# MP-Gadget/MP-Gadget

Hardware: AMD Instinct MI355X
Metric: particle-updates/sec (gravity force step: PM + tree build + short-range walk) (higher is better)
Workload: dtype f64

## Files before the change

include/mpgadget_hip.h:

```cpp
#ifndef MPGADGET_HIP_H
#define MPGADGET_HIP_H

#include <stddef.h>
#include <stdint.h>

#ifdef __cplusplus
extern "C" {
#endif

typedef struct mpg_engine mpg_engine;

int mpg_engine_create(mpg_engine **out, int device);
void mpg_engine_destroy(mpg_engine *eng);
const char *mpg_last_error(void);
const char *mpg_version(void);
const char *mpg_build_stamp(void);
int mpg_engine_set_stream(mpg_engine *eng, void *hip_stream);
void *mpg_engine_get_stream(mpg_engine *eng);
int mpg_engine_synchronize(mpg_engine *eng);

typedef struct mpg_gravshort_tree_params {
    double ErrTolForceAcc;
    double BHOpeningAngle;
    double MaxBHOpeningAngle;
// ... 295 lines not shown
int mpg_domain_local_refine(const uint64_t *keys, const int64_t *costs, int64_t nsample, mpg_topnode *tree, int *size, int MaxTopNodes, int *failed);
int mpg_domain_toptree_truncate(mpg_topnode *tree, int *size, int64_t countlimit, int64_t costlimit);
int mpg_domain_toptree_merge(mpg_topnode *A, int *sizeA, const mpg_topnode *B, int sizeB, int MaxTopNodes, int *failed);
int mpg_domain_global_refine(mpg_topnode *tree, int *size, int MaxTopNodes, int64_t countlimit, int64_t costlimit, int *failed);
int mpg_domain_create_topleaves(mpg_topnode *tree, int size, int *leaf_topnode, int *nleaves);
int mpg_domain_assign_topleaves_balanced(mpg_topnode *tree, int size, int *leaf_topnode, int nleaves, const int64_t *cost, int NTask,
                                         int NsegmentPerTask, int *leaf_task, int *StartLeaf, int *EndLeaf);
int mpg_dev_domain_topleaves(mpg_engine *eng, int64_t n, const double *d_pos, const unsigned char *d_garbage, double BoxSize,
                             const mpg_topnode *tree, int size, int nleaves, const int *leaf_task, int NTask, int32_t *d_topleaf,
                             int32_t *d_task, int64_t *leaf_counts, int64_t *task_counts);

int mpg_dev_peano_keys(mpg_engine *eng, int64_t n, const double *d_pos, double BoxSize, uint64_t *d_keys);
int mpg_dev_order_by_type_and_key(mpg_engine *eng, int64_t n, const unsigned char *d_type, const unsigned char *d_flags,
                                  const uint64_t *d_keys, int *d_perm, int64_t *n_live);

typedef struct mpg_fof_params {
    int FOFPrimaryLinkTypes;
    int FOFSecondaryLinkTypes;
    double FOFHaloComovingLinkingLength;
    int FOFHaloMinLength;
} mpg_fof_params;
typedef struct mpg_fof_groups {
    uint64_t *MinID;
    int *Length, *GrNr, *LenType;
    double *Mass, *MassType;
    double *CM, *Vel, *Jmom;
    double *Imom;
    float *FirstPos;
} mpg_fof_groups;
int mpg_dev_fof_fof(mpg_engine *eng, const mpg_fof_params *par, const uint64_t *d_id, const double *d_vel, const double *d_hsml,
                    const unsigned char *d_flags, int64_t *d_grnr, int64_t *ngroups);
int mpg_dev_fof_groups(mpg_engine *eng, const mpg_fof_groups *out);

typedef struct mpg_bigblock_info {
    char dtype[8];
    int nmemb;
    int nfile;
    int64_t size;
} mpg_bigblock_info;
int mpg_bigfile_block_info(const char *file, const char *block, mpg_bigblock_info *info);
int mpg_bigfile_read_block(const char *file, const char *block, int64_t start, int64_t count, const char *want_dtype, void *out);
int mpg_bigfile_write_block(const char *file, const char *block, const char *dtype, int nmemb, int nfile, int64_t size, const char *src_dtype,
                            const void *data);
int mpg_bigfile_get_attr(const char *file, const char *block, const char *name, const char *want_dtype, void *out, int nmemb);
int mpg_bigfile_set_attr(const char *file, const char *block, const char *name, const char *dtype, const void *data, int nmemb);

int mpg_gravpm_measure_power(mpg_engine *eng, int on);
int mpg_dev_gravpm_powerspectrum_raw(mpg_engine *eng, double *d_acc, int64_t *d_modes);
int mpg_powerspectrum_sum(int nbins, const double *acc, const int64_t *modes, double BoxSize_in_MPC, double *kk, double *Power,
                          int64_t *Nmodes, int *nonzero);
int mpg_gravpm_get_powerspectrum(mpg_engine *eng, double BoxSize_in_MPC, double *kk, double *Power, int64_t *Nmodes, int *nonzero);
int mpg_powerspectrum_save(const char *OutputDir, const char *filename, double Time, double D1, int nonzero, const double *kk,
                           const double *Power, const int64_t *Nmodes);

int mpg_dev_pm_slab_init(mpg_engine *eng, int rank, int world, int64_t *cplx_per_peer, int64_t *plane_doubles);

int mpg_dev_tree_top_partial(mpg_engine *eng, int La, int64_t n_own, double *d_out);
int mpg_dev_tree_top_set(mpg_engine *eng, int La, const double *d_sums);
int mpg_dev_pm_slab_forward_a(mpg_engine *eng, double *sendA);
int mpg_dev_pm_slab_forward_b(mpg_engine *eng, double *recvA, double *sendB);
int mpg_dev_pm_slab_inverse_c(mpg_engine *eng, const double *recvB, double *ghost_send);
int mpg_dev_pm_slab_readout(mpg_engine *eng, const double *ghost_recv, const int *d_targets, int64_t ntargets, double *d_gravpm,
                            double *d_potential);

typedef struct mpg_comm {
    void *ctx;
    int ThisTask, NTask;
    int device_buffers;
    int (*allreduce)(void *ctx, void *buf, int64_t count, int dtype, int op, int on_device);
    int (*alltoall_i64)(void *ctx, const int64_t *send, int64_t *recv);
    int (*alltoallv)(void *ctx, const void *send, const int64_t *sendbytes, const int64_t *sdispls, void *recv, const int64_t *recvbytes,
                     const int64_t *rdispls, int on_device);
    int (*bind_stream)(void *ctx, void *hip_stream);
} mpg_comm;

#define MPG_RCCL_ID_BYTES 128
typedef struct mpg_rccl mpg_rccl;
int mpg_rccl_available(void);
int mpg_rccl_get_unique_id(void *id128);
int mpg_rccl_create(mpg_rccl **out, int ThisTask, int NTask, const void *id128, int device);
int mpg_rccl_comm(mpg_rccl *r, mpg_comm *out);
int mpg_rccl_selftest(mpg_rccl *r, int64_t bytes_per_peer);
int mpg_rccl_stats(mpg_rccl *r, int64_t *calls3, int64_t *bytes_sent, int *version);
int mpg_rccl_comm_info(mpg_rccl *r, int *nranks, int *rank, int *device);
const char *mpg_rccl_last_error(mpg_rccl *r);
void mpg_rccl_destroy(mpg_rccl *r);

typedef struct mpg_dist mpg_dist;
int mpg_dist_create(mpg_dist **out, mpg_engine *eng, const mpg_comm *comm);
void mpg_dist_destroy(mpg_dist *d);
int mpg_dist_domain_decompose(mpg_dist *d, int64_t n, const double *d_pos, const unsigned char *d_garbage, double BoxSize,
                              int DomainOverDecompositionFactor, int DomainUseGlobalSorting, const float *d_cost, int *NTopNodes,
                              int *NTopLeaves);
int mpg_dist_domain_get(mpg_dist *d, mpg_topnode *TopNodes, int *leaf_task, int *StartLeaf, int *EndLeaf, int64_t *TopLeafCount);
int mpg_dist_domain_exchange(mpg_dist *d, int64_t n, int ncols, const void *const *d_cols, const int *col_bytes, int64_t *n_new,
                             void **d_new_cols);
int mpg_dist_use_decomposition(mpg_dist *d, double BoxSize, double margin, int La);
int mpg_dist_domain_maintain(mpg_dist *d, int64_t n, const double *d_pos, const unsigned char *d_garbage, double BoxSize, int64_t *n_leaving);
int mpg_dist_set_domain(mpg_dist *d, double BoxSize, const mpg_topnode *TopNodes, int NTopNodes, const int *leaf_task, int NTopLeaves,
                        double margin, int La);
int mpg_dist_gravity_step(mpg_dist *d, int64_t n_own, const double *d_pos, const float *d_mass, const double *d_oldacc,
                          const double *d_prev_accel, double *d_accel, double *d_gravpm, double *d_potential, double rho0);
int mpg_dist_dev_gravpm_force(mpg_dist *d, int64_t n_own, const double *d_pos, const float *d_mass, double *d_gravpm, double *d_potential);
int mpg_dist_dev_set_garbage(mpg_dist *d, int64_t n_own, const unsigned char *d_garbage);
int mpg_dist_dev_force_tree_build(mpg_dist *d, int64_t n_own, const double *d_pos, const float *d_mass);
int mpg_dist_dev_grav_short_tree(mpg_dist *d, const double *d_oldacc, const double *d_prev_accel, const double *d_gravpm, double *d_accel,
// ... 47 lines not shown
```

mp-gadget_amd/build.py:

```python
import hashlib
import os
import subprocess
import sys
from concurrent.futures import ThreadPoolExecutor

HERE = os.path.dirname(os.path.abspath(__file__))
CSRC = os.path.join(HERE, "csrc")
OBJ = os.path.join(CSRC, "_obj")
LIB = os.path.join(HERE, "libmpgadget_hip.so")
SOURCES = ["tree_build.hip", "grav_walk.hip", "grav_walk_coop.hip", "grav_walk_split.hip", "grav_pair_walk.hip", "pm.hip", "sph.hip", "timestep.hip", "peano.hip", "domain.hip", "fof.hip", "snapshot_io.hip", "engine.hip", "dist.hip", "rccl_comm.hip"]
HIPCC = os.environ.get("HIPCC", "/opt/rocm/bin/hipcc")
FLAGS = ["--offload-arch=gfx950", "-O3", "-std=c++17", "-fPIC", "-Wall", "-Wno-unused-function", "-Wno-unused-result"]
_EXTRA = os.environ.get("MPG_EXTRA_FLAGS", "")
_EXTRA_FILE, _EXTRA = (_EXTRA.split(":", 1) if ".hip:" in _EXTRA else ("", _EXTRA))


def _headers():
    hs = sorted(os.path.join(CSRC, f) for f in os.listdir(CSRC) if f.endswith(".h"))
    hs.append(os.path.join(HERE, "..", "include", "mpgadget_hip.h"))
    return hs


def _sha(paths, extra=""):
    h = hashlib.sha256(extra.encode())
    for p in paths:
        h.update(os.path.basename(p).encode())
        with open(p, "rb") as f:
            h.update(f.read())
    return h.hexdigest()


def source_stamp():
    return _sha([os.path.join(CSRC, s) for s in SOURCES] + _headers(), " ".join(FLAGS) + os.environ.get("MPG_EXTRA_FLAGS", ""))[:32]


def _read(path):
    try:
        with open(path) as f:
            return f.read().strip()
    except OSError:
        return ""


def build(force=False, verbose=False):
    os.makedirs(OBJ, exist_ok=True)
    headers = _headers()

    def compile_one(src):
        s = os.path.join(CSRC, src)
        o = os.path.join(OBJ, src.replace(".hip", ".o"))
        flags = FLAGS + (_EXTRA.split() if _EXTRA_FILE in ("", src) else [])
        want = _sha([s] + headers, " ".join(flags))
        if force or not os.path.exists(o) or _read(o + ".hash") != want:
            cmd = [HIPCC] + flags + ["-c", s, "-o", o]
            if verbose:
                print(" ".join(cmd))
            subprocess.check_call(cmd)
            with open(o + ".hash", "w") as f:
                f.write(want)
            return o, True
        return o, False

    with ThreadPoolExecutor(max_workers=4) as ex:
# ... 22 lines not shown
```

mp-gadget_amd/csrc/engine.hip:

```cpp
#include "engine_internal.h"
#include <atomic>
#include <chrono>
#include <cstdio>

static thread_local std::string g_err;
std::string &mpg_err_slot() { return g_err; }

extern "C" {

const char *mpg_last_error(void) { return g_err.c_str(); }
const char *mpg_version(void) { return "mpgadget_hip 0.1 (gfx950; TreePM gravity: PM + tree + short-range walk)"; }

int mpg_engine_create(mpg_engine **out, int device)
{
    API_BEGIN
    MPG_CHECK(out != nullptr, "mpg_engine_create: null output pointer");
    int ndev = 0;
    hipError_t e = hipGetDeviceCount(&ndev);
    if(e != hipSuccess || ndev <= 0)
        fail(__FILE__, __LINE__, "mpg_engine_create: no HIP device available (this engine has no CPU path)");
    MPG_CHECK(device >= 0 && device < ndev, "mpg_engine_create: bad device index");
    MPG_HIP(hipSetDevice(device));
    mpg_engine *eng = new mpg_engine();
    eng->device = device;
// ... 191 lines not shown
    API_BEGIN
    MPG_CHECK(eng, "null engine");
    MPG_CHECK(n >= 0 && (n == 0 || (d_pos && d_mass)), "mpg_dev_bind_particles: null particle arrays");
    MPG_CHECK(BoxSize > 0, "mpg_dev_bind_particles: BoxSize must be positive");
    eng->host_join();
    eng->n = n;
    eng->d_pos = d_pos;
    eng->d_mass = d_mass;
    eng->d_type = d_type;
    eng->box = BoxSize;
    eng->pm_queued = false;
    API_END
}

int mpg_dev_gravpm_force(mpg_engine *eng, double *d_gravpm, double *d_potential)
{
    API_BEGIN
    MPG_CHECK(eng && d_gravpm, "null argument");
    MPG_HIP(hipSetDevice(eng->device));
    MPG_CHECK(eng->pm.nmesh > 0, "gravpm_force called before gravpm_init_periodic");
    MPG_CHECK(eng->pm.box == eng->box, "gravpm_force: BoxSize of the mesh differs from the bound particles");
    static const bool no_overlap = getenv("MPG_NO_TREE_OVERLAP") != nullptr;
    if(!no_overlap && !eng->timer.enabled) {
        if(!eng->aux_stream) {
            MPG_HIP(hipStreamCreateWithFlags(&eng->aux_stream, hipStreamNonBlocking));
            MPG_HIP(hipEventCreateWithFlags(&eng->ev_inputs, hipEventDisableTiming));
            MPG_HIP(hipEventCreateWithFlags(&eng->ev_tree_done, hipEventDisableTiming));
            MPG_HIP(hipEventCreateWithFlags(&eng->ev_pad_done, hipEventDisableTiming));
        }
        MPG_HIP(hipEventRecord(eng->ev_inputs, eng->stream));
        eng->pm_queued = true;
    }
    eng->pm.force(eng->n, eng->d_pos, eng->d_mass, nullptr, d_gravpm, d_potential, eng->stream, &eng->timer);
    API_END
}

int mpg_dev_tree_top_partial(mpg_engine *eng, int La, int64_t n_own, double *d_out)
{
    API_BEGIN
    MPG_CHECK(eng && d_out, "null argument");
    MPG_CHECK(eng->tree_allocated, "no tree");
    MPG_HIP(hipSetDevice(eng->device));
    eng->tree.top_partial(La, n_own, d_out, eng->stream);
    API_END
}

int mpg_dev_tree_top_set(mpg_engine *eng, int La, const double *d_sums)
{
    API_BEGIN
    MPG_CHECK(eng && d_sums, "null argument");
    MPG_CHECK(eng->tree_allocated, "no tree");
    MPG_HIP(hipSetDevice(eng->device));
    eng->tree.top_set(La, d_sums, eng->stream);
    API_END
}

int mpg_dev_pm_slab_init(mpg_engine *eng, int rank, int world, int64_t *cplx_per_peer, int64_t *plane_doubles)
{
    API_BEGIN
    MPG_CHECK(eng, "null engine");
    MPG_HIP(hipSetDevice(eng->device));
    eng->pm.slab_init(rank, world);
    if(cplx_per_peer)
        *cplx_per_peer = (int64_t)eng->pm.slab_cplx_per_peer();
    if(plane_doubles)
        *plane_doubles = (int64_t)eng->pm.nmesh * eng->pm.nmesh;
    API_END
}

int mpg_dev_pm_slab_forward_a(mpg_engine *eng, double *sendA)
{
    API_BEGIN
    MPG_CHECK(eng && sendA, "null argument");
    MPG_HIP(hipSetDevice(eng->device));
    MPG_CHECK(eng->pm.box == eng->box, "gravpm_force: BoxSize of the mesh differs from the bound particles");
    eng->pm.slab_forward_a(eng->n, eng->d_pos, eng->d_mass, sendA, eng->stream);
    API_END
}

int mpg_dev_pm_slab_forward_b(mpg_engine *eng, double *recvA, double *sendB)
{
    API_BEGIN
    MPG_CHECK(eng && recvA && sendB, "null argument");
    MPG_HIP(hipSetDevice(eng->device));
    eng->pm.slab_forward_b(recvA, sendB, eng->stream);
    API_END
}

int mpg_dev_pm_slab_inverse_c(mpg_engine *eng, const double *recvB, double *ghost_send)
{
    API_BEGIN
    MPG_CHECK(eng && recvB && ghost_send, "null argument");
    MPG_HIP(hipSetDevice(eng->device));
    eng->pm.slab_inverse_c(recvB, ghost_send, eng->stream);
    API_END
}

int mpg_dev_pm_slab_readout(mpg_engine *eng, const double *ghost_recv, const int *d_targets, int64_t ntargets, double *d_gravpm,
                            double *d_potential)
{
    API_BEGIN
    MPG_CHECK(eng && ghost_recv && d_gravpm && (d_targets || ntargets == 0), "null argument");
    MPG_HIP(hipSetDevice(eng->device));
    eng->pm.slab_readout(ghost_recv, d_targets, ntargets, eng->d_pos, d_gravpm, d_potential, eng->stream);
    API_END
}
// ... 2769 lines not shown
```

mp-gadget_amd/csrc/pm.h:

```cpp
#pragma once
#include "mpg_common.h"
#include "tree_build.h"
#include <rocfft/rocfft.h>
#include <vector>

namespace mpg {

struct FftPlan {
    rocfft_plan plan = nullptr;
    rocfft_execution_info info = nullptr;
    DevBuf<char> work;
    void create(rocfft_result_placement placement, rocfft_transform_type type, int dims, const size_t *lengths, size_t batch,
                const size_t *in_strides = nullptr, size_t in_dist = 0, const size_t *out_strides = nullptr, size_t out_dist = 0);
    void exec(void *in, void *out, hipStream_t st);
    void destroy();
    bool ready() const { return plan != nullptr; }
};

struct PMesh {
    double box = 0, Asmth = 0, G = 0, cellsize = 0;
    int nmesh = 0;
    bool have_plans = false;
    bool kspace_force = false;
    FftPlan plan_r2c, plan_c2r;
    DevBuf<double> real;
    DevBuf<double> rho_k;
    DevBuf<double> work_k;
    DevBuf<double> grad_z;
    DevBuf<double> invsinc2, difffac;
    struct DepositState {
        int mode = 0, since_tune = 0;
    } dep_single, dep_slab;
    void deposit(int64_t n, const double *d_pos, const float *d_mass, const uint8_t *d_active, double *mesh, int x0, int P, DepositState &ds,
                 hipStream_t st, EventTimer *tm);
    DevBuf<unsigned long long> dep_keys_a, dep_keys_b;
    DevBuf<int> dep_idx_a, dep_idx_b;
    DevBuf<char> dep_tmp;
    bool measure_power = true, ps_valid = false;
    DevBuf<double> ps_acc;
    DevBuf<unsigned long long> ps_modes;
    void ps_zero(hipStream_t st);
    size_t ps_lds_bytes() const { return (size_t)nmesh * 3 * sizeof(double); }

    void init(double BoxSize, double Asmth, int Nmesh, double G, hipStream_t st);
    void ensure_single();
    void destroy();
    void force(int64_t n, const double *d_pos, const float *d_mass, const uint8_t *d_active, double *d_gravpm, double *d_potential,
               hipStream_t st, EventTimer *tm);
    ~PMesh() { destroy(); }

    struct Slab {
        int rank = 0, world = 1, P = 0, Py = 0;
        bool ready = false;
        FftPlan p2d_r2c, p2d_c2r, p1d_fwd, p1d_inv, p1d_fwd_t, p1d_inv_t;
        bool strided = false;
        DevBuf<double> phi;
        DevBuf<double> force;
        DevBuf<double> C;
        DevBuf<double> rho_k;
        DevBuf<double> work;
    } slab;
    DevBuf<unsigned> slab_err;
    size_t slab_cplx_per_peer() const { return (size_t)slab.P * slab.Py * (nmesh / 2 + 1); }
    void slab_init(int rank, int world);
    void slab_destroy();
    void slab_forward_a(int64_t n, const double *d_pos, const float *d_mass, double *sendA, hipStream_t st);
    void slab_forward_b(double *recvA, double *sendB, hipStream_t st);
    void slab_inverse_c(const double *recvB, double *ghost_send, hipStream_t st);
    void slab_readout_rows(const double *ghost_recv, int64_t nrows, const double *d_pos, double *d_gravpm, double *d_potential, hipStream_t st);
    void slab_readout(const double *ghost_recv, const int *targets, int64_t nt, const double *d_pos, double *d_gravpm, double *d_potential,
                      hipStream_t st);
};

}
```

mp-gadget_amd/csrc/pm.hip:

```cpp
#include "pm.h"
#include <cmath>
#include <cstdlib>
#include <cstring>
#include <rocprim/rocprim.hpp>

namespace mpg {

#define MPG_FFT(expr)                                                                                          \
    do {                                                                                                       \
        rocfft_status _r = (expr);                                                                             \
        if(_r != rocfft_status_success)                                                                        \
            ::mpg::fail(__FILE__, __LINE__, std::string("rocFFT error ") + std::to_string((int)_r) + " in " #expr); \
    } while(0)

__device__ __forceinline__ int wrap(int i, int n)
{
    i = (i >= n) ? i - n : i;
    i = (i < 0) ? i + n : i;
    return i;
}

__global__ void __launch_bounds__(256) k_cic_deposit(int64_t n, const double *__restrict__ pos, const float *__restrict__ mass,
                                                     const uint8_t *__restrict__ active, double cellsize, int nmesh,
                                                     double *__restrict__ mesh)
// ... 444 lines not shown

void FftPlan::create(rocfft_result_placement placement, rocfft_transform_type type, int dims, const size_t *lengths, size_t batch,
                     const size_t *in_strides, size_t in_dist, const size_t *out_strides, size_t out_dist)
{
    static const bool once = (rocfft_setup(), true);
    (void)once;
    destroy();
    rocfft_plan_description desc = nullptr;
    if(in_strides || out_strides) {
        MPG_FFT(rocfft_plan_description_create(&desc));
        const bool real_fwd = type == rocfft_transform_type_real_forward, real_inv = type == rocfft_transform_type_real_inverse;
        const rocfft_array_type in_t = real_fwd ? rocfft_array_type_real : (real_inv ? rocfft_array_type_hermitian_interleaved : rocfft_array_type_complex_interleaved);
        const rocfft_array_type out_t = real_fwd ? rocfft_array_type_hermitian_interleaved : (real_inv ? rocfft_array_type_real : rocfft_array_type_complex_interleaved);
        MPG_FFT(rocfft_plan_description_set_data_layout(desc, in_t, out_t, nullptr, nullptr, in_strides ? (size_t)dims : 0, in_strides, in_dist,
                                                        out_strides ? (size_t)dims : 0, out_strides, out_dist));
    }
    MPG_FFT(rocfft_plan_create(&plan, placement, type, rocfft_precision_double, (size_t)dims, lengths, batch, desc));
    if(desc)
        MPG_FFT(rocfft_plan_description_destroy(desc));
    MPG_FFT(rocfft_execution_info_create(&info));
    size_t wb = 0;
    MPG_FFT(rocfft_plan_get_work_buffer_size(plan, &wb));
    if(wb > 0) {
        work.reserve(wb + 64);
        MPG_FFT(rocfft_execution_info_set_work_buffer(info, work.p, wb));
    }
}

void FftPlan::exec(void *in, void *out, hipStream_t st)
{
    MPG_FFT(rocfft_execution_info_set_stream(info, st));
    void *ib[1] = {in}, *ob[1] = {out};
    MPG_FFT(rocfft_execute(plan, ib, out == in ? nullptr : ob, info));
}

void FftPlan::destroy()
{
    if(info)
        (void)rocfft_execution_info_destroy(info);
    if(plan)
        (void)rocfft_plan_destroy(plan);
    info = nullptr;
    plan = nullptr;
    work.release();
}

void PMesh::ensure_single()
{
    if(have_plans)
        return;
    const size_t nreal = (size_t)nmesh * nmesh * nmesh;
    const size_t ncplx = (size_t)nmesh * nmesh * (nmesh / 2 + 1);
    real.reserve(nreal);
    rho_k.reserve(2 * ncplx);
    work_k.reserve(2 * ncplx);
    const size_t len3[3] = {(size_t)nmesh, (size_t)nmesh, (size_t)nmesh};
    plan_r2c.create(rocfft_placement_notinplace, rocfft_transform_type_real_forward, 3, len3, 1);
    plan_c2r.create(rocfft_placement_notinplace, rocfft_transform_type_real_inverse, 3, len3, 1);
    have_plans = true;
}

void PMesh::ps_zero(hipStream_t st)
{
    ps_acc.reserve(2 * (size_t)nmesh + 8);
    ps_modes.reserve((size_t)nmesh + 8);
    MPG_HIP(hipMemsetAsync(ps_acc.p, 0, (2 * (size_t)nmesh + 1) * sizeof(double), st));
    MPG_HIP(hipMemsetAsync(ps_modes.p, 0, (size_t)nmesh * sizeof(unsigned long long), st));
    ps_valid = true;
}

void PMesh::destroy()
{
    if(have_plans) {
        plan_r2c.destroy();
        plan_c2r.destroy();
        have_plans = false;
    }
    slab_destroy();
    real.release();
    rho_k.release();
    work_k.release();
    grad_z.release();
    nmesh = 0;
}

__global__ void k_cic_deposit_slab(int64_t n, const double *__restrict__ pos, const float *__restrict__ mass, double cellsize, int nmesh, int x0,
                                   int P, double *__restrict__ slab);

void PMesh::deposit(int64_t n, const double *d_pos, const float *d_mass, const uint8_t *d_active, double *mesh, int x0, int P, DepositState &ds,
                    hipStream_t st, EventTimer *tm)
{
    const size_t ncell = (size_t)P * nmesh * nmesh, nreal = (size_t)nmesh * nmesh * nmesh;
    const bool whole = x0 == 0 && P == nmesh;
    auto plain = [&]() {
        if(whole)
            hipLaunchKernelGGL(k_cic_deposit, dim3(nblk(n)), dim3(256), 0, st, n, d_pos, d_mass, d_active, cellsize, nmesh, mesh);
        else
            hipLaunchKernelGGL(k_cic_deposit_slab, dim3(nblk(n)), dim3(256), 0, st, n, d_pos, d_mass, cellsize, nmesh, x0, P, mesh);
    };
    auto sorted = [&]() {
        dep_keys_a.reserve((size_t)n + 1);
        dep_keys_b.reserve((size_t)n + 1);
        dep_idx_a.reserve((size_t)n + 1);
        dep_idx_b.reserve((size_t)n + 1);
        hipLaunchKernelGGL(k_cell_keys, dim3(nblk(n)), dim3(256), 0, st, n, d_pos, d_active, cellsize, nmesh, dep_keys_a.p, dep_idx_a.p);
        int bits = 1;
        while(bits < 64 && ((unsigned long long)1 << bits) < (unsigned long long)nreal)
            bits++;
        size_t tb = 0;
        MPG_HIP(rocprim::radix_sort_pairs(nullptr, tb, dep_keys_a.p, dep_keys_b.p, dep_idx_a.p, dep_idx_b.p, (size_t)n, 0, 64, st));
        dep_tmp.reserve(tb + 16);
        MPG_HIP(rocprim::radix_sort_pairs((void *)dep_tmp.p, tb, dep_keys_a.p, dep_keys_b.p, dep_idx_a.p, dep_idx_b.p, (size_t)n, 0,
                                          d_active ? 64 : bits, st));
        hipLaunchKernelGGL(k_cic_deposit_sorted, dim3(nblk(n)), dim3(256), 0, st, n, dep_keys_b.p, dep_idx_b.p, d_pos, d_mass, cellsize, nmesh, x0, P,
                           mesh);
    };
    if(const char *e = getenv("MPG_PM_DEPOSIT"))
        ds.mode = !strcmp(e, "sorted") ? 2 : 1;
    if(ds.mode == 0 || ++ds.since_tune >= 64) {
        hipEvent_t e0, e1, e2;
        MPG_HIP(hipEventCreate(&e0));
        MPG_HIP(hipEventCreate(&e1));
        MPG_HIP(hipEventCreate(&e2));
        MPG_HIP(hipEventRecord(e0, st));
        sorted();
        MPG_HIP(hipEventRecord(e1, st));
        MPG_HIP(hipMemsetAsync(mesh, 0, ncell * sizeof(double), st));
        plain();
        MPG_HIP(hipEventRecord(e2, st));
        MPG_HIP(hipEventSynchronize(e2));
        float ts = 0, tp = 0;
        MPG_HIP(hipEventElapsedTime(&ts, e0, e1));
        MPG_HIP(hipEventElapsedTime(&tp, e1, e2));
        (void)hipEventDestroy(e0);
        (void)hipEventDestroy(e1);
        (void)hipEventDestroy(e2);
        ds.mode = ts < tp ? 2 : 1;
        ds.since_tune = 0;
        if(tm)
            tm->start(st);
        MPG_HIP(hipMemsetAsync(mesh, 0, ncell * sizeof(double), st));
    }
    if(ds.mode == 2)
        sorted();
    else
        plain();
}

void PMesh::force(int64_t n, const double *d_pos, const float *d_mass, const uint8_t *d_active, double *d_gravpm, double *d_potential,
                  hipStream_t st, EventTimer *tm)
{
    MPG_CHECK(nmesh > 0, "gravpm_force called before gravpm_init_periodic");
    MPG_CHECK(!slab.ready, "gravpm_force: the mesh is in its slab-decomposed form (use the pm_slab calls)");
    ensure_single();
    const size_t nreal = (size_t)nmesh * nmesh * nmesh;
    const size_t ncplx = (size_t)nmesh * nmesh * (nmesh / 2 + 1);
    float t_fft = 0, t_tr = 0, t_ro = 0, t;
    if(tm)
        tm->start(st);
    MPG_HIP(hipMemsetAsync(real.p, 0, nreal * sizeof(double), st));
    if(n > 0)
        deposit(n, d_pos, d_mass, d_active, real.p, 0, nmesh, dep_single, st, tm);
    if(tm)
        tm->lap(st, &tm->t.pm_deposit);
    plan_r2c.exec(real.p, rho_k.p, st);
    if(tm) {
        tm->lap(st, &t);
        t_fft += t;
    }
    const double asmth2 = pow((2 * M_PI) * Asmth / nmesh, 2);
    const double pot_factor = -G / (M_PI * box);
    static const bool fuse_ps = !(getenv("MPG_PM_FUSE_PS") && getenv("MPG_PM_FUSE_PS")[0] == '0');
    if(measure_power && fuse_ps) {
        ps_zero(st);
        hipLaunchKernelGGL((k_power_spectrum<false, true>), dim3(2048), dim3(256), ps_lds_bytes(), st, nmesh, nmesh, 0, invsinc2.p, (double2 *)rho_k.p,
                           ps_acc.p, ps_modes.p, asmth2, pot_factor);
    }
    else {
        if(measure_power) {
            ps_zero(st);
            hipLaunchKernelGGL((k_power_spectrum<false, false>), dim3(2048), dim3(256), ps_lds_bytes(), st, nmesh, nmesh, 0, invsinc2.p,
                               (double2 *)rho_k.p, ps_acc.p, ps_modes.p, 0.0, 0.0);
        }
        hipLaunchKernelGGL(k_potential_transfer<false>, dim3(nblk(ncplx)), dim3(256), 0, st, nmesh, nmesh, 0, asmth2, pot_factor, invsinc2.p,
                           (double2 *)rho_k.p);
    }
    if(tm) {
        tm->lap(st, &t);
        t_tr += t;
    }
    if(!kspace_force) {
        plan_c2r.exec(rho_k.p, real.p, st);
        if(tm) {
            tm->lap(st, &t);
            t_fft += t;
        }
        static const bool one_pass = !(getenv("MPG_PM_GRADIENT_PASSES") && getenv("MPG_PM_GRADIENT_PASSES")[0] == '3');
        static const bool stencil = one_pass && !(getenv("MPG_PM_STENCIL") && getenv("MPG_PM_STENCIL")[0] == '0');
        if(stencil) {
            if(n > 0)
                hipLaunchKernelGGL(k_cic_readout_stencil, dim3(nblk(n)), dim3(256), 0, st, n, d_pos, d_active, cellsize, nmesh, (double)nmesh / box,
                                   (const double *)real.p, d_gravpm, d_potential);
            if(tm) {
                tm->lap(st, &t);
                t_ro += t;
            }
        }
        else {
        if(n > 0 && d_potential)
            hipLaunchKernelGGL(k_cic_readout, dim3(nblk(n)), dim3(256), 0, st, n, d_pos, d_active, cellsize, nmesh, real.p, 3, d_potential);
        if(tm) {
            tm->lap(st, &t);
            t_ro += t;
        }
        if(one_pass) {
            grad_z.reserve(nreal);
            double *g[3] = {work_k.p, rho_k.p, grad_z.p};
            hipLaunchKernelGGL(k_gradient3, dim3(nblk(nreal)), dim3(256), 0, st, nmesh, (double)nmesh / box, real.p, g[0], g[1], g[2]);
            if(tm) {
                tm->lap(st, &t);
                t_tr += t;
            }
            for(int axis = 0; axis < 3 && n > 0; axis++)
                hipLaunchKernelGGL(k_cic_readout, dim3(nblk(n)), dim3(256), 0, st, n, d_pos, d_active, cellsize, nmesh, g[axis], axis, d_gravpm);
            if(tm) {
                tm->lap(st, &t);
                t_ro += t;
            }
        }
        else
            for(int axis = 0; axis < 3; axis++) {
                hipLaunchKernelGGL(k_gradient_axis, dim3(nblk(nreal)), dim3(256), 0, st, nmesh, nmesh, axis, (double)nmesh / box, real.p, work_k.p, 0);
                if(tm) {
                    tm->lap(st, &t);
                    t_tr += t;
                }
                if(n > 0)
                    hipLaunchKernelGGL(k_cic_readout, dim3(nblk(n)), dim3(256), 0, st, n, d_pos, d_active, cellsize, nmesh, work_k.p, axis, d_gravpm);
                if(tm) {
                    tm->lap(st, &t);
                    t_ro += t;
                }
            }
        }
    }
    else
        for(int f = 0; f < 4; f++) {
        const int axis = f - 1;
// ... 397 lines not shown
```

mp-gadget_amd/engine.py:

```python
import ctypes as C
import os

import numpy as np

_HERE = os.path.dirname(os.path.abspath(__file__))
LIB_PATH = os.path.join(_HERE, "libmpgadget_hip.so")
TABLE_PATH = os.path.join(_HERE, "data", "shortrange_force_kernels.f64")

PARTICLE_DTYPE = np.dtype({
    "names": ["Pos", "TopLeaf", "Mass", "PI", "Flags", "TimeBinHydro", "TimeBinGravity", "Type", "Vel",
              "FullTreeGravAccel", "GravPM", "Ti_drift", "Hsml", "DtHsml", "ID", "GrNr", "Potential"],
    "formats": [("<f8", 3), "<i4", "<f4", "<i4", "u1", "u1", "u1", "u1", ("<f8", 3), ("<f8", 3), ("<f8", 3), "<i8", "<f8",
                "<f8", "<u8", "<i8", "<f8"],
    "offsets": [0, 24, 28, 32, 36, 37, 38, 39, 40, 64, 88, 112, 120, 128, 136, 144, 152],
    "itemsize": 160})

SHORTRANGE_FORCE_WINDOW_TYPE_EXACT = 0
SHORTRANGE_FORCE_WINDOW_TYPE_ERFC = 1
ALLMASK, GASMASK, DMMASK, NUMASK, STARMASK, BHMASK = 63, 1, 2, 4, 16, 32


class EngineError(RuntimeError):
    pass

# ... 556 lines not shown
        return ng.value

    def dev_fof_groups(self, ngroups, device="cuda"):
        import torch
        mk = lambda shape, dt: torch.zeros(shape, dtype=dt, device=device)
        g = dict(MinID=mk(ngroups, torch.int64), Length=mk(ngroups, torch.int32), GrNr=mk(ngroups, torch.int32),
                 LenType=mk((ngroups, 6), torch.int32), Mass=mk(ngroups, torch.float64), MassType=mk((ngroups, 6), torch.float64),
                 CM=mk((ngroups, 3), torch.float64), Vel=mk((ngroups, 3), torch.float64), Jmom=mk((ngroups, 3), torch.float64),
                 Imom=mk((ngroups, 3, 3), torch.float64), FirstPos=mk((ngroups, 3), torch.float32))
        out = FofGroupsC(*[g[k].data_ptr() for k in ("MinID", "Length", "GrNr", "LenType", "Mass", "MassType", "CM", "Vel", "Jmom", "Imom", "FirstPos")])
        self._ck(self.lib.mpg_dev_fof_groups(self.h, C.byref(out)))
        return g

    @staticmethod
    def _hier_arrays(vel, gravpm, fulltree_accel, tb_grav, potential=None, flags=None, stored_accel=None):
        dp = lambda t: None if t is None else t.data_ptr()
        return HierGravArrays(dp(vel), dp(gravpm), dp(fulltree_accel), dp(potential), dp(tb_grav), dp(flags), dp(stored_accel))

    def dev_build_active_sublist(self, active, tb_grav, flags, maxtimebin, Ti_Current, out):
        n = C.c_int64(0)
        na = active.shape[0] if active is not None else tb_grav.shape[0]
        self._ck(self.lib.mpg_dev_build_active_sublist(self.h, _ptr(active), C.c_int64(na), _ptr(tb_grav), _ptr(flags), int(maxtimebin),
                                                       C.c_int64(Ti_Current), _ptr(out), C.byref(n)))
        return n.value

    def dev_hierarchical_gravity_and_timesteps(self, arrays, active, num_active_gravity, times, sync_loga, ErrTolIntAccuracy, MinSizeTimestep,
                                               atime, hubble, dti_max_pm, rho0, gravkick, HybridNuGrav=0):
        loga = (C.c_double * len(sync_loga))(*[float(x) for x in sync_loga])
        tl = Timeline(len(sync_loga), C.cast(loga, C.POINTER(C.c_double)))
        par = TimestepParams(ErrTolIntAccuracy, MinSizeTimestep)
        fn = GRAVKICK_FN(lambda ctx, a, b: float(gravkick(a, b)))
        bad = C.c_int64(0)
        na = active.shape[0] if active is not None else 0
        nag = num_active_gravity if active is not None else 0
        self._ck(self.lib.mpg_dev_hierarchical_gravity_and_timesteps(self.h, C.byref(arrays), _ptr(active), C.c_int64(na), C.c_int64(nag),
                                                                     C.byref(times), C.byref(tl), C.byref(par), C.c_double(atime),
                                                                     C.c_double(hubble), C.c_int64(dti_max_pm), C.c_double(rho0),
                                                                     int(HybridNuGrav), fn, None, C.byref(bad)))
        return bad.value

    def dev_hierarchical_gravity_accelerations(self, arrays, active, num_active_gravity, times, rho0, gravkick, HybridNuGrav=0):
        fn = GRAVKICK_FN(lambda ctx, a, b: float(gravkick(a, b)))
        na = active.shape[0] if active is not None else 0
        nag = num_active_gravity if active is not None else 0
        self._ck(self.lib.mpg_dev_hierarchical_gravity_accelerations(self.h, C.byref(arrays), _ptr(active), C.c_int64(na), C.c_int64(nag),
                                                                     C.byref(times), C.c_double(rho0), int(HybridNuGrav), fn, None))

    def dev_tree_top_partial(self, La, n_own, out):
        self._ck(self.lib.mpg_dev_tree_top_partial(self.h, int(La), C.c_int64(n_own), _ptr(out)))

    def dev_tree_top_set(self, La, sums):
        self._ck(self.lib.mpg_dev_tree_top_set(self.h, int(La), _ptr(sums)))

    def dev_pm_slab_init(self, rank, world):
        a, b = C.c_int64(0), C.c_int64(0)
        self._ck(self.lib.mpg_dev_pm_slab_init(self.h, int(rank), int(world), C.byref(a), C.byref(b)))
        return a.value, b.value

    def dev_pm_slab_forward_a(self, sendA):
        self._ck(self.lib.mpg_dev_pm_slab_forward_a(self.h, _ptr(sendA)))

    def dev_pm_slab_forward_b(self, recvA, sendB):
        self._ck(self.lib.mpg_dev_pm_slab_forward_b(self.h, _ptr(recvA), _ptr(sendB)))

    def dev_pm_slab_inverse_c(self, recvB, ghost_send):
        self._ck(self.lib.mpg_dev_pm_slab_inverse_c(self.h, _ptr(recvB), _ptr(ghost_send)))

    def dev_pm_slab_readout(self, ghost_recv, targets, gravpm, potential=None):
        self._ck(self.lib.mpg_dev_pm_slab_readout(self.h, _ptr(ghost_recv), _ptr(targets), C.c_int64(targets.shape[0]), _ptr(gravpm),
                                                  _ptr(potential)))

    def dev_force_tree_build(self, mask=ALLMASK):
        self._ck(self.lib.mpg_dev_force_tree_build(self.h, int(mask)))

    def dev_grav_short_tree(self, accel, oldacc=None, prev_accel=None, gravpm=None, active=None, potential=None, rho0=0.0,
                            nactive=None):
        if active is None:
            nact = 0
        elif nactive is not None:
            nact = int(nactive)
        else:
            nact = active.shape[0]
        self._ck(self.lib.mpg_dev_grav_short_tree(self.h, _ptr(oldacc), _ptr(prev_accel), _ptr(gravpm), _ptr(active),
                                                  C.c_int64(nact), _ptr(accel), _ptr(potential), C.c_double(rho0)))

    def set_densitypar(self, DensityResolutionEta=1.0, MaxNumNgbDeviation=2.0, BlackHoleNgbFactor=2.0,
                       BlackHoleMaxAccretionRadius=99999., DensityKernelType=DENSITY_KERNEL_QUINTIC_SPLINE,
                       MinGasHsmlFractional=0.006):
        p = DensityParams(DensityResolutionEta, MaxNumNgbDeviation, BlackHoleNgbFactor, BlackHoleMaxAccretionRadius,
                          DensityKernelType, MinGasHsmlFractional)
        self._ck(self.lib.mpg_set_densitypar(self.h, C.byref(p)))

    def set_hydropar(self, DensityIndependentSphOn=1, DensityContrastLimit=100.0, ArtBulkViscConst=0.75):
        p = HydroParams(DensityIndependentSphOn, DensityContrastLimit, ArtBulkViscConst)
        self._ck(self.lib.mpg_set_hydropar(self.h, C.byref(p)))

    def GetNumNgb(self):
        return self.lib.mpg_get_numngb(self.h)

    @staticmethod
    def _sph_arrays(arrays):
        a = SphArraysC()
        for k in SPH_ARRAY_FIELDS:
            t = arrays.get(k)
            setattr(a, k, None if t is None else (t if isinstance(t, int) else t.data_ptr()))
        return a
# ... 132 lines not shown
```

Before: 241.4 million.

## Replace rocFFT 3D PM transform with custom column FFTs fused with Green's function

```diff
diff --git a/include/mpgadget_hip.h b/include/mpgadget_hip.h
--- a/include/mpgadget_hip.h
+++ b/include/mpgadget_hip.h
@@ -371,6 +371,8 @@
 int mpg_gravpm_get_powerspectrum(mpg_engine *eng, double BoxSize_in_MPC, double *kk, double *Power, int64_t *Nmodes, int *nonzero);
 int mpg_powerspectrum_save(const char *OutputDir, const char *filename, double Time, double D1, int nonzero, const double *kk,
                            const double *Power, const int64_t *Nmodes);
+
+int mpg_dev_pm_transform(mpg_engine *eng, int dir, double *d_real, double *d_cplx);
 
 int mpg_dev_pm_slab_init(mpg_engine *eng, int rank, int world, int64_t *cplx_per_peer, int64_t *plane_doubles);
 
diff --git a/mp-gadget_amd/build.py b/mp-gadget_amd/build.py
--- a/mp-gadget_amd/build.py
+++ b/mp-gadget_amd/build.py
@@ -8,7 +8,7 @@
 CSRC = os.path.join(HERE, "csrc")
 OBJ = os.path.join(CSRC, "_obj")
 LIB = os.path.join(HERE, "libmpgadget_hip.so")
-SOURCES = ["tree_build.hip", "grav_walk.hip", "grav_walk_coop.hip", "grav_walk_split.hip", "grav_pair_walk.hip", "pm.hip", "sph.hip", "timestep.hip", "peano.hip", "domain.hip", "fof.hip", "snapshot_io.hip", "engine.hip", "dist.hip", "rccl_comm.hip"]
+SOURCES = ["tree_build.hip", "grav_walk.hip", "grav_walk_coop.hip", "grav_walk_split.hip", "grav_pair_walk.hip", "pm.hip", "pm_fft.hip", "sph.hip", "timestep.hip", "peano.hip", "domain.hip", "fof.hip", "snapshot_io.hip", "engine.hip", "dist.hip", "rccl_comm.hip"]
 HIPCC = os.environ.get("HIPCC", "/opt/rocm/bin/hipcc")
 FLAGS = ["--offload-arch=gfx950", "-O3", "-std=c++17", "-fPIC", "-Wall", "-Wno-unused-function", "-Wno-unused-result"]
 _EXTRA = os.environ.get("MPG_EXTRA_FLAGS", "")
diff --git a/mp-gadget_amd/csrc/engine.hip b/mp-gadget_amd/csrc/engine.hip
--- a/mp-gadget_amd/csrc/engine.hip
+++ b/mp-gadget_amd/csrc/engine.hip
@@ -267,6 +267,15 @@
     MPG_CHECK(eng->tree_allocated, "no tree");
     MPG_HIP(hipSetDevice(eng->device));
     eng->tree.top_set(La, d_sums, eng->stream);
+    API_END
+}
+
+int mpg_dev_pm_transform(mpg_engine *eng, int dir, double *d_real, double *d_cplx)
+{
+    API_BEGIN
+    MPG_CHECK(eng && d_real && d_cplx && dir != 0, "null argument");
+    MPG_HIP(hipSetDevice(eng->device));
+    eng->pm.transform(dir, d_real, d_cplx, eng->stream);
     API_END
 }
 
diff --git a/mp-gadget_amd/csrc/pm.h b/mp-gadget_amd/csrc/pm.h
--- a/mp-gadget_amd/csrc/pm.h
+++ b/mp-gadget_amd/csrc/pm.h
@@ -44,6 +44,18 @@
 
     void init(double BoxSize, double Asmth, int Nmesh, double G, hipStream_t st);
     void ensure_single();
+    void ensure_plans3d();
+
+    bool have_colfft = false;
+    int colfft_cus = 1;
+    FftPlan plan_z_r2c, plan_z_c2r;
+    DevBuf<double> twiddle;
+    static bool colfft_supported(int n);
+    bool colfft_selected() const;
+    void ensure_colfft(hipStream_t st);
+    void colfft_pass(int what, double *cplx, double asmth2, double pot_factor, hipStream_t st);
+    void colfft_solve(double asmth2, double pot_factor, hipStream_t st);
+    void transform(int dir, double *d_real, double *d_cplx, hipStream_t st);
     void destroy();
     void force(int64_t n, const double *d_pos, const float *d_mass, const uint8_t *d_active, double *d_gravpm, double *d_potential,
                hipStream_t st, EventTimer *tm);
diff --git a/mp-gadget_amd/csrc/pm.hip b/mp-gadget_amd/csrc/pm.hip
--- a/mp-gadget_amd/csrc/pm.hip
+++ b/mp-gadget_amd/csrc/pm.hip
@@ -520,8 +520,15 @@
     const size_t nreal = (size_t)nmesh * nmesh * nmesh;
     const size_t ncplx = (size_t)nmesh * nmesh * (nmesh / 2 + 1);
     real.reserve(nreal);
-    rho_k.reserve(2 * ncplx);
+    const size_t ncplx_pad = colfft_supported(nmesh) ? (size_t)nmesh * nmesh * ((nmesh / 2 + 8) / 8 * 8) : ncplx;
+    rho_k.reserve(2 * std::max(ncplx, ncplx_pad));
     work_k.reserve(2 * ncplx);
+}
+
+void PMesh::ensure_plans3d()
+{
+    if(have_plans)
+        return;
     const size_t len3[3] = {(size_t)nmesh, (size_t)nmesh, (size_t)nmesh};
     plan_r2c.create(rocfft_placement_notinplace, rocfft_transform_type_real_forward, 3, len3, 1);
     plan_c2r.create(rocfft_placement_notinplace, rocfft_transform_type_real_inverse, 3, len3, 1);
@@ -543,6 +550,12 @@
         plan_r2c.destroy();
         plan_c2r.destroy();
         have_plans = false;
+    }
+    if(have_colfft) {
+        plan_z_r2c.destroy();
+        plan_z_c2r.destroy();
+        twiddle.release();
+        have_colfft = false;
     }
     slab_destroy();
     real.release();
@@ -631,37 +644,50 @@
         deposit(n, d_pos, d_mass, d_active, real.p, 0, nmesh, dep_single, st, tm);
     if(tm)
         tm->lap(st, &tm->t.pm_deposit);
-    plan_r2c.exec(real.p, rho_k.p, st);
-    if(tm) {
-        tm->lap(st, &t);
-        t_fft += t;
-    }
     const double asmth2 = pow((2 * M_PI) * Asmth / nmesh, 2);
     const double pot_factor = -G / (M_PI * box);
-    static const bool fuse_ps = !(getenv("MPG_PM_FUSE_PS") && getenv("MPG_PM_FUSE_PS")[0] == '0');
-    if(measure_power && fuse_ps) {
-        ps_zero(st);
-        hipLaunchKernelGGL((k_power_spectrum<false, true>), dim3(2048), dim3(256), ps_lds_bytes(), st, nmesh, nmesh, 0, invsinc2.p, (double2 *)rho_k.p,
-                           ps_acc.p, ps_modes.p, asmth2, pot_factor);
-    }
-    else {
-        if(measure_power) {
-            ps_zero(st);
-            hipLaunchKernelGGL((k_power_spectrum<false, false>), dim3(2048), dim3(256), ps_lds_bytes(), st, nmesh, nmesh, 0, invsinc2.p,
-                               (double2 *)rho_k.p, ps_acc.p, ps_modes.p, 0.0, 0.0);
-        }
-        hipLaunchKernelGGL(k_potential_transfer<false>, dim3(nblk(ncplx)), dim3(256), 0, st, nmesh, nmesh, 0, asmth2, pot_factor, invsinc2.p,
-                           (double2 *)rho_k.p);
-    }
-    if(tm) {
-        tm->lap(st, &t);
-        t_tr += t;
-    }
-    if(!kspace_force) {
-        plan_c2r.exec(rho_k.p, real.p, st);
+    const bool colfft = colfft_selected();
+    if(colfft) {
+        colfft_solve(asmth2, pot_factor, st);
         if(tm) {
             tm->lap(st, &t);
             t_fft += t;
+        }
+    }
+    else {
+        ensure_plans3d();
+        plan_r2c.exec(real.p, rho_k.p, st);
+        if(tm) {
+            tm->lap(st, &t);
+            t_fft += t;
+        }
+        static const bool fuse_ps = !(getenv("MPG_PM_FUSE_PS") && getenv("MPG_PM_FUSE_PS")[0] == '0');
+        if(measure_power && fuse_ps) {
+            ps_zero(st);
+            hipLaunchKernelGGL((k_power_spectrum<false, true>), dim3(2048), dim3(256), ps_lds_bytes(), st, nmesh, nmesh, 0, invsinc2.p, (double2 *)rho_k.p,
+                               ps_acc.p, ps_modes.p, asmth2, pot_factor);
+        }
+        else {
+            if(measure_power) {
+                ps_zero(st);
+                hipLaunchKernelGGL((k_power_spectrum<false, false>), dim3(2048), dim3(256), ps_lds_bytes(), st, nmesh, nmesh, 0, invsinc2.p,
+                                   (double2 *)rho_k.p, ps_acc.p, ps_modes.p, 0.0, 0.0);
+            }
+            hipLaunchKernelGGL(k_potential_transfer<false>, dim3(nblk(ncplx)), dim3(256), 0, st, nmesh, nmesh, 0, asmth2, pot_factor, invsinc2.p,
+                               (double2 *)rho_k.p);
+        }
+        if(tm) {
+            tm->lap(st, &t);
+            t_tr += t;
+        }
+    }
+    if(!kspace_force) {
+        if(!colfft) {
+            plan_c2r.exec(rho_k.p, real.p, st);
+            if(tm) {
+                tm->lap(st, &t);
+                t_fft += t;
+            }
         }
         static const bool one_pass = !(getenv("MPG_PM_GRADIENT_PASSES") && getenv("MPG_PM_GRADIENT_PASSES")[0] == '3');
         static const bool stencil = one_pass && !(getenv("MPG_PM_STENCIL") && getenv("MPG_PM_STENCIL")[0] == '0');
diff --git a/mp-gadget_amd/csrc/pm_fft.hip b/mp-gadget_amd/csrc/pm_fft.hip
--- /dev/null
+++ b/mp-gadget_amd/csrc/pm_fft.hip
@@ -0,0 +1,354 @@
+#include "pm.h"
+#include <cmath>
+#include <cstdlib>
+#include <cstring>
+
+namespace mpg {
+
+static constexpr int FFT_THREADS = 256;
+static constexpr int FUSED_THREADS = 512;
+
+template <int N> struct FftCols {
+    static constexpr int C = N >= 1024 ? 4 : 8;
+};
+
+static inline int nzp_of(int nmesh) { return ((nmesh / 2 + 1) + 7) / 8 * 8; }
+
+__device__ __forceinline__ double2 cmul(double2 a, double2 b) { return make_double2(a.x * b.x - a.y * b.y, a.x * b.y + a.y * b.x); }
+__device__ __forceinline__ double2 cadd(double2 a, double2 b) { return make_double2(a.x + b.x, a.y + b.y); }
+__device__ __forceinline__ double2 csub(double2 a, double2 b) { return make_double2(a.x - b.x, a.y - b.y); }
+template <int DIR> __device__ __forceinline__ double2 mul_mi(double2 a) { return DIR < 0 ? make_double2(a.y, -a.x) : make_double2(-a.y, a.x); }
+
+template <int R, int DIR> __device__ __forceinline__ void dft(double2 *v)
+{
+    if constexpr(R == 2) {
+        const double2 a = v[0], b = v[1];
+        v[0] = cadd(a, b);
+        v[1] = csub(a, b);
+    }
+    else if constexpr(R == 4) {
+        const double2 s02 = cadd(v[0], v[2]), d02 = csub(v[0], v[2]);
+        const double2 s13 = cadd(v[1], v[3]), d13 = mul_mi<DIR>(csub(v[1], v[3]));
+        v[0] = cadd(s02, s13);
+        v[2] = csub(s02, s13);
+        v[1] = cadd(d02, d13);
+        v[3] = csub(d02, d13);
+    }
+    else {
+        double2 e[4] = {v[0], v[2], v[4], v[6]}, o[4] = {v[1], v[3], v[5], v[7]};
+        dft<4, DIR>(e);
+        dft<4, DIR>(o);
+        const double c = 0.70710678118654752440;
+        const double2 o1 = make_double2(c * (o[1].x - DIR * o[1].y), c * (o[1].y + DIR * o[1].x));
+        const double2 o2 = mul_mi<DIR>(o[2]);
+        const double2 o3 = make_double2(-c * (o[3].x + DIR * o[3].y), c * (DIR * o[3].x - o[3].y));
+        v[0] = cadd(e[0], o[0]);
+        v[4] = csub(e[0], o[0]);
+        v[1] = cadd(e[1], o1);
+        v[5] = csub(e[1], o1);
+        v[2] = cadd(e[2], o2);
+        v[6] = csub(e[2], o2);
+        v[3] = cadd(e[3], o3);
+        v[7] = csub(e[3], o3);
+    }
+}
+
+template <int N, int C, int DIR, int NS, int TPB = FFT_THREADS>
+__device__ __forceinline__ void fft_passes(double2 *t, const double2 *__restrict__ tw)
+{
+    constexpr int R = (N / NS) >= 8 ? 8 : N / NS;
+    constexpr int NB = C * (N / R);
+    constexpr int IT = (NB + TPB - 1) / TPB;
+    double2 v[IT][R];
+#pragma unroll
+    for(int it = 0; it < IT; it++) {
+        const int b = threadIdx.x + it * TPB;
+        if(NB % TPB == 0 || b < NB) {
+            const int c = b % C, j = b / C;
+#pragma unroll
+            for(int r = 0; r < R; r++)
+                v[it][r] = t[(j + r * (N / R)) * C + c];
+        }
+    }
+    __syncthreads();
+#pragma unroll
+    for(int it = 0; it < IT; it++) {
+        const int b = threadIdx.x + it * TPB;
+        if(NB % TPB == 0 || b < NB) {
+            const int c = b % C, j = b / C;
+            const int k = j % NS;
+            if constexpr(NS > 1) {
+#pragma unroll
+                for(int r = 1; r < R; r++) {
+                    double2 w = tw[r * k * (N / (NS * R))];
+                    if(DIR > 0)
+                        w.y = -w.y;
+                    v[it][r] = cmul(v[it][r], w);
+                }
+            }
+            dft<R, DIR>(v[it]);
+            const int o = (j / NS) * NS * R + k;
+#pragma unroll
+            for(int r = 0; r < R; r++)
+                t[(o + r * NS) * C + c] = v[it][r];
+        }
+    }
+    __syncthreads();
+    if constexpr(NS * R < N)
+        fft_passes<N, C, DIR, NS * R, TPB>(t, tw);
+}
+
+template <int N, int C, int TPB = FFT_THREADS> __device__ __forceinline__ void tile_load(double2 *t, const double2 *__restrict__ g, size_t S)
+{
+    constexpr int E = (N * C + TPB - 1) / TPB;
+    double2 v[E];
+#pragma unroll
+    for(int i = 0; i < E; i++) {
+        const int e = threadIdx.x + i * TPB;
+        if((N * C) % TPB == 0 || e < N * C)
+            v[i] = g[(size_t)(e / C) * S + (e % C)];
+    }
+#pragma unroll
+    for(int i = 0; i < E; i++) {
+        const int e = threadIdx.x + i * TPB;
+        if((N * C) % TPB == 0 || e < N * C)
+            t[e] = v[i];
+    }
+    __syncthreads();
+}
+
+template <int N, int C, int TPB = FFT_THREADS> __device__ __forceinline__ void tile_store(const double2 *t, double2 *__restrict__ g, size_t S)
+{
+    constexpr int E = (N * C + TPB - 1) / TPB;
+#pragma unroll
+    for(int i = 0; i < E; i++) {
+        const int e = threadIdx.x + i * TPB;
+        if((N * C) % TPB == 0 || e < N * C)
+            g[(size_t)(e / C) * S + (e % C)] = t[e];
+    }
+}
+
+template <int N, int DIR>
+__global__ void __launch_bounds__(FFT_THREADS) k_fft_cols(double2 *__restrict__ cplx, int ngroups, size_t ostride, size_t S,
+                                                          const double2 *__restrict__ tw)
+{
+    constexpr int C = FftCols<N>::C;
+    __shared__ double2 t[N * C];
+    const int o = blockIdx.x / ngroups, g = blockIdx.x % ngroups;
+    double2 *base = cplx + (size_t)o * ostride + (size_t)g * C;
+    tile_load<N, C>(t, base, S);
+    fft_passes<N, C, DIR, 1>(t, tw);
+    tile_store<N, C>(t, base, S);
+}
+
+template <int N, bool MEASURE>
+__global__ void __launch_bounds__(FUSED_THREADS) k_fft_x_fused(double2 *__restrict__ cplx, int ngroups, const double2 *__restrict__ tw,
+                                                             const double *__restrict__ invsinc2, double asmth2, double pot_factor,
+                                                             double *__restrict__ acc, unsigned long long *__restrict__ modes)
+{
+    constexpr int C = FftCols<N>::C;
+    constexpr int nbins = N;
+    constexpr int NZ = N / 2 + 1;
+    __shared__ double2 t[N * C];
+    __shared__ double s_pow[MEASURE ? nbins : 1], s_kk[MEASURE ? nbins : 1];
+    __shared__ unsigned long long s_n[MEASURE ? nbins : 1];
+    if constexpr(MEASURE)
+        for(int b = threadIdx.x; b < nbins; b += FUSED_THREADS) {
+            s_pow[b] = 0;
+            s_kk[b] = 0;
+            s_n[b] = 0;
+        }
+    const size_t S = (size_t)N * ngroups * C;
+    const int ntiles = N * ngroups;
+    const double binsperunit = (nbins - 1) / log(sqrt(3.0) * N / 2.0);
+    for(int tile = blockIdx.x; tile < ntiles; tile += gridDim.x) {
+        const int iy = tile / ngroups, g = tile % ngroups;
+        double2 *base = cplx + (size_t)iy * ngroups * C + (size_t)g * C;
+        tile_load<N, C, FUSED_THREADS>(t, base, S);
+        fft_passes<N, C, -1, 1, FUSED_THREADS>(t, tw);
+        const int ky = iy <= N / 2 ? iy : iy - N;
+#pragma unroll 1
+        for(int e = threadIdx.x; e < N * C; e += FUSED_THREADS) {
+            const int ix = e / C, iz = g * C + e % C;
+            if(iz >= NZ) {
+                t[e] = make_double2(0.0, 0.0);
+                continue;
+            }
+            const int kx = ix <= N / 2 ? ix : ix - N;
+            const int kz = iz;
+            const long long k2 = (long long)kx * kx + (long long)ky * ky + (long long)kz * kz;
+            const double2 v = t[e];
+            if(k2 == 0) {
+                if constexpr(MEASURE)
+                    acc[2 * nbins] = v.x * v.x + v.y * v.y;
+                t[e] = make_double2(0.0, 0.0);
+                continue;
+            }
+            const double f = invsinc2[ix] * invsinc2[iy] * invsinc2[iz];
+            const double smth = exp(-(double)k2 * asmth2) / (double)k2;
+            const double fac = pot_factor * smth * f * f;
+            t[e] = make_double2(v.x * fac, v.y * fac);
+            if constexpr(MEASURE) {
+                const double m = v.x * v.x + v.y * v.y;
+                const int kint = (int)floor(binsperunit * log((double)k2) / 2.);
+                if(kint >= nbins)
+                    continue;
+                const int w = (kz == 0 || kz == N / 2) ? 1 : 2;
+                __hip_atomic_fetch_add(&s_pow[kint], w * m * f * f, __ATOMIC_RELAXED, __HIP_MEMORY_SCOPE_WORKGROUP);
+                __hip_atomic_fetch_add(&s_kk[kint], w * sqrt((double)k2), __ATOMIC_RELAXED, __HIP_MEMORY_SCOPE_WORKGROUP);
+                __hip_atomic_fetch_add(&s_n[kint], (unsigned long long)w, __ATOMIC_RELAXED, __HIP_MEMORY_SCOPE_WORKGROUP);
+            }
+        }
+        __syncthreads();
+        fft_passes<N, C, +1, 1, FUSED_THREADS>(t, tw);
+        tile_store<N, C, FUSED_THREADS>(t, base, S);
+        __syncthreads();
+    }
+    if constexpr(MEASURE) {
+        __syncthreads();
+        for(int b = threadIdx.x; b < nbins; b += FUSED_THREADS)
+            if(s_n[b]) {
+                unsafeAtomicAdd(&acc[b], s_pow[b]);
+                unsafeAtomicAdd(&acc[nbins + b], s_kk[b]);
+                atomicAdd(&modes[b], s_n[b]);
+            }
+    }
+}
+
+
+bool PMesh::colfft_supported(int n) { return n >= 16 && n <= 1024 && (n & (n - 1)) == 0; }
+
+bool PMesh::colfft_selected() const
+{
+    if(kspace_force || !colfft_supported(nmesh))
+        return false;
+    const char *e = getenv("MPG_PM_FFT");
+    return !(e && !strcmp(e, "rocfft"));
+}
+
+void PMesh::ensure_colfft(hipStream_t st)
+{
+    if(have_colfft)
+        return;
+    const int nzp = nzp_of(nmesh);
+    const size_t len = (size_t)nmesh, unit = 1, batch = (size_t)nmesh * nmesh;
+    plan_z_r2c.create(rocfft_placement_notinplace, rocfft_transform_type_real_forward, 1, &len, batch, &unit, (size_t)nmesh, &unit, (size_t)nzp);
+    plan_z_c2r.create(rocfft_placement_notinplace, rocfft_transform_type_real_inverse, 1, &len, batch, &unit, (size_t)nzp, &unit, (size_t)nmesh);
+    std::vector<double> w(2 * (size_t)nmesh);
+    for(int k = 0; k < nmesh; k++) {
+        const long double a = -2.0L * 3.141592653589793238462643383279502884L * (long double)k / (long double)nmesh;
+        w[2 * k] = (double)cosl(a);
+        w[2 * k + 1] = (double)sinl(a);
+    }
+    twiddle.reserve(2 * (size_t)nmesh);
+    MPG_HIP(hipMemcpyAsync(twiddle.p, w.data(), w.size() * sizeof(double), hipMemcpyHostToDevice, st));
+    MPG_HIP(hipStreamSynchronize(st));
+    int dev = 0, ncu = 0;
+    MPG_HIP(hipGetDevice(&dev));
+    MPG_HIP(hipDeviceGetAttribute(&ncu, hipDeviceAttributeMultiprocessorCount, dev));
+    colfft_cus = ncu > 0 ? ncu : 1;
+    have_colfft = true;
+}
+
+template <int N>
+static void colfft_launch(int what, double2 *cplx, const double2 *tw, const double *invsinc2, double asmth2, double pot_factor, double *acc,
+                          unsigned long long *modes, int ncu, hipStream_t st)
+{
+    const int nzp = nzp_of(N), ng = nzp / FftCols<N>::C;
+    const size_t plane = (size_t)N * nzp;
+    switch(what) {
+    case 0:
+        hipLaunchKernelGGL((k_fft_cols<N, -1>), dim3(N * ng), dim3(FFT_THREADS), 0, st, cplx, ng, plane, (size_t)nzp, tw);
+        break;
+    case 1:
+        hipLaunchKernelGGL((k_fft_cols<N, +1>), dim3(N * ng), dim3(FFT_THREADS), 0, st, cplx, ng, plane, (size_t)nzp, tw);
+        break;
+    case 2:
+        hipLaunchKernelGGL((k_fft_cols<N, -1>), dim3(N * ng), dim3(FFT_THREADS), 0, st, cplx, ng, (size_t)nzp, plane, tw);
+        break;
+    case 3:
+        hipLaunchKernelGGL((k_fft_cols<N, +1>), dim3(N * ng), dim3(FFT_THREADS), 0, st, cplx, ng, (size_t)nzp, plane, tw);
+        break;
+    default: {
+        auto kern = what == 4 ? k_fft_x_fused<N, true> : k_fft_x_fused<N, false>;
+        int per_cu = 0;
+        MPG_HIP(hipOccupancyMaxActiveBlocksPerMultiprocessor(&per_cu, kern, FUSED_THREADS, 0));
+        const int ntiles = N * ng;
+        const int grid = std::min(ntiles, ncu * std::max(per_cu, 1));
+        hipLaunchKernelGGL(kern, dim3(grid), dim3(FUSED_THREADS), 0, st, cplx, ng, tw, invsinc2, asmth2, pot_factor, acc, modes);
+    }
+    }
+}
+
+void PMesh::colfft_pass(int what, double *cplx, double asmth2, double pot_factor, hipStream_t st)
+{
+    const double2 *tw = (const double2 *)twiddle.p;
+    double2 *c = (double2 *)cplx;
+    const int ncu = colfft_cus;
+    switch(nmesh) {
+#define MPG_COLFFT_CASE(NN)                                                                                                  \
+    case NN:                                                                                                                 \
+        colfft_launch<NN>(what, c, tw, invsinc2.p, asmth2, pot_factor, ps_acc.p, ps_modes.p, ncu, st);                        \
+        break;
+        MPG_COLFFT_CASE(16)
+        MPG_COLFFT_CASE(32)
+        MPG_COLFFT_CASE(64)
+        MPG_COLFFT_CASE(128)
+        MPG_COLFFT_CASE(256)
+        MPG_COLFFT_CASE(512)
+        MPG_COLFFT_CASE(1024)
+#undef MPG_COLFFT_CASE
+    default:
+        fail(__FILE__, __LINE__, "column FFT: unsupported Nmesh " + std::to_string(nmesh));
+    }
+    MPG_HIP(hipGetLastError());
+}
+
+void PMesh::colfft_solve(double asmth2, double pot_factor, hipStream_t st)
+{
+    ensure_colfft(st);
+    plan_z_r2c.exec(real.p, rho_k.p, st);
+    colfft_pass(0, rho_k.p, 0, 0, st);
+    if(measure_power)
+        ps_zero(st);
+    colfft_pass(measure_power ? 4 : 5, rho_k.p, asmth2, pot_factor, st);
+    colfft_pass(1, rho_k.p, 0, 0, st);
+    plan_z_c2r.exec(rho_k.p, real.p, st);
+}
+
+void PMesh::transform(int dir, double *d_real, double *d_cplx, hipStream_t st)
+{
+    MPG_CHECK(nmesh > 0, "pm_transform called before gravpm_init_periodic");
+    MPG_CHECK(!slab.ready, "pm_transform: the mesh is in its slab-decomposed form");
+    ensure_single();
+    const size_t nz = (size_t)nmesh / 2 + 1, rows = (size_t)nmesh * nmesh;
+    if(!colfft_selected()) {
+        ensure_plans3d();
+        if(dir > 0)
+            plan_r2c.exec(d_real, d_cplx, st);
+        else {
+            MPG_HIP(hipMemcpyAsync(work_k.p, d_cplx, rows * nz * 2 * sizeof(double), hipMemcpyDeviceToDevice, st));
+            plan_c2r.exec(work_k.p, d_real, st);
+        }
+        return;
+    }
+    ensure_colfft(st);
+    const size_t nzp = (size_t)nzp_of(nmesh);
+    if(dir > 0) {
+        plan_z_r2c.exec(d_real, rho_k.p, st);
+        colfft_pass(0, rho_k.p, 0, 0, st);
+        colfft_pass(2, rho_k.p, 0, 0, st);
+        MPG_HIP(hipMemcpy2DAsync(d_cplx, nz * 2 * sizeof(double), rho_k.p, nzp * 2 * sizeof(double), nz * 2 * sizeof(double), rows,
+                                 hipMemcpyDeviceToDevice, st));
+    }
+    else {
+        MPG_HIP(hipMemsetAsync(rho_k.p, 0, rows * nzp * 2 * sizeof(double), st));
+        MPG_HIP(hipMemcpy2DAsync(rho_k.p, nzp * 2 * sizeof(double), d_cplx, nz * 2 * sizeof(double), nz * 2 * sizeof(double), rows,
+                                 hipMemcpyDeviceToDevice, st));
+        colfft_pass(3, rho_k.p, 0, 0, st);
+        colfft_pass(1, rho_k.p, 0, 0, st);
+        plan_z_c2r.exec(rho_k.p, d_real, st);
+    }
+}
+
+}
diff --git a/mp-gadget_amd/engine.py b/mp-gadget_amd/engine.py
--- a/mp-gadget_amd/engine.py
+++ b/mp-gadget_amd/engine.py
@@ -632,6 +632,9 @@
     def dev_tree_top_set(self, La, sums):
         self._ck(self.lib.mpg_dev_tree_top_set(self.h, int(La), _ptr(sums)))
 
+    def dev_pm_transform(self, direction, real, cplx):
+        self._ck(self.lib.mpg_dev_pm_transform(self.h, int(direction), _ptr(real), _ptr(cplx)))
+
     def dev_pm_slab_init(self, rank, world):
         a, b = C.c_int64(0), C.c_int64(0)
         self._ck(self.lib.mpg_dev_pm_slab_init(self.h, int(rank), int(world), C.byref(a), C.byref(b)))
```

New measurement: 244.9 million (median of 6 runs). 1.5% higher.
